# xuyuan/waymo_2d_tracking

Hardware: AMD Instinct MI355X
Metric: end-to-end frames/sec (detect+SORT) on 1920x1280 Waymo frames (higher is better)
Workload: dtype f32; 1 GPU; Cascade R-CNN X152-32x8d-FPN dconv (random-init, fp32, batch 1) on synthetic 1920x1280x3 frames -> top-100 detections/frame -> SORT (max_age 2, min_hits 0, all boxes tracked; trackers resident for the whole segment); 5 cameras x 2 frames per step per GPU; 1x1 and dense 3x3 convolutions: f32 operands as exact 3 x bf16 splits, six cross terms on the bf16 matrix cores, f32 accumulate (csrc/det_gemm_s; stage=e2e, parallelism=sequence-shard x1

## Files before the change

waymo_2d_tracking_amd/csrc/det_deform.hip:

```cpp
#include "common.h"
#include "../../include/waymodet.h"
#include <cstdlib>

namespace {

using f32x4 = __attribute__((ext_vector_type(4))) float;
constexpr int TP = 64;
constexpr int CCH = 128;
constexpr int LDC = CCH + 2;

struct Sample {
    unsigned idx[4];
    float wgt[4];
};

template <int CG, bool DEFORM>
__global__ __launch_bounds__(256, (CG <= 32 ? 3 : 2)) void deform_conv3x3_kernel(
    const float* __restrict__ x, const float* __restrict__ offset, const float* __restrict__ mask,
    const float* __restrict__ wp, const float* __restrict__ scale, const float* __restrict__ bias, int relu,
    int batch, int H, int W, int C, int Cout, int Ho, int Wo, int stride, int pad, float* __restrict__ y) {
    constexpr bool PRIV = CG <= 32;
    constexpr int LDW = PRIV ? 34 : LDC;
    __shared__ Sample tab[TP * 9];
    __shared__ __attribute__((aligned(16))) float col[PRIV ? 4 * TP * 34 : TP * LDC];
    const int tid = threadIdx.x, lane = tid & 63, wave = tid >> 6;
    const int tiles_x = (Wo + 7) >> 3, tiles_y = (Ho + 7) >> 3;
    const int ntiles = batch * tiles_y * tiles_x;
    const int nchunks = C / CCH;
    int tile, chunk;
    {
        const int b = blockIdx.x;
        const int xcd = b & 7, slot = b >> 3;
        if (nchunks >= 8 && (nchunks & 7) == 0) {
            const int cpx = nchunks >> 3;
            chunk = xcd * cpx + slot % cpx;
            tile = slot / cpx;
        } else if (nchunks < 8 && (8 % nchunks) == 0 && (ntiles % (8 / nchunks)) == 0) {
            const int xpc = 8 / nchunks;
            const int tpp = ntiles / xpc;
            chunk = xcd / xpc;
            tile = (xcd % xpc) * tpp + slot;
        } else {
            chunk = b / ntiles;
            tile = b - chunk * ntiles;
        }
    }
    if (tile >= ntiles || chunk >= nchunks) return;
    const int tn = tile / (tiles_y * tiles_x);
    const int trem = tile - tn * tiles_y * tiles_x;
    const int tyy = trem / tiles_x, txx = trem - tyy * tiles_x;
    __shared__ int pix[TP];
    if (tid < TP) {
        const int ho = tyy * 8 + (tid >> 3), wo = txx * 8 + (tid & 7);
        pix[tid] = (ho < Ho && wo < Wo) ? (tn * Ho + ho) * Wo + wo : -1;
    }
    __syncthreads();
    const int c0 = chunk * CCH;
    for (int e = tid; e < TP * 9; e += 256) {
        const int p = e / 9, k = e - 9 * p;
        const long gp = pix[p];
        Sample s;
#pragma unroll
        for (int q = 0; q < 4; ++q) { s.idx[q] = 0u; s.wgt[q] = 0.f; }
        if (gp >= 0) {
            const int n = (int)(gp / ((long)Ho * Wo));
            const int rem = (int)(gp - (long)n * Ho * Wo);
            const int ho = rem / Wo, wo = rem - ho * Wo;
            const int kh = k / 3, kw = k - 3 * kh;
            if (!DEFORM) {
                const int hi = ho * stride - pad + kh, wi = wo * stride - pad + kw;
                if (hi >= 0 && hi < H && wi >= 0 && wi < W) { s.idx[0] = (unsigned)(n * H * W + hi * W + wi) * (unsigned)C * 4u; s.wgt[0] = 1.f; }
                tab[e] = s;
                continue;
            }
            const float* off = offset + (size_t)gp * 18;
            const float h_im = (float)(ho * stride - pad + kh) + off[2 * k];
            const float w_im = (float)(wo * stride - pad + kw) + off[2 * k + 1];
            if (h_im > -1.f && w_im > -1.f && h_im < (float)H && w_im < (float)W) {
                const int hl = (int)floorf(h_im), wl = (int)floorf(w_im);
                const int hh = hl + 1, wh = wl + 1;
                const float lh = h_im - (float)hl, lw = w_im - (float)wl;
                const float uh = 1.f - lh, uw = 1.f - lw;
                const float m = mask ? mask[(size_t)gp * 9 + k] : 1.f;
                const int base = n * H * W;
                if (hl >= 0 && wl >= 0) { s.idx[0] = (unsigned)(base + hl * W + wl) * (unsigned)C * 4u; s.wgt[0] = uh * uw * m; }
                if (hl >= 0 && wh <= W - 1) { s.idx[1] = (unsigned)(base + hl * W + wh) * (unsigned)C * 4u; s.wgt[1] = uh * lw * m; }
                if (hh <= H - 1 && wl >= 0) { s.idx[2] = (unsigned)(base + hh * W + wl) * (unsigned)C * 4u; s.wgt[2] = lh * uw * m; }
                if (hh <= H - 1 && wh <= W - 1) { s.idx[3] = (unsigned)(base + hh * W + wh) * (unsigned)C * 4u; s.wgt[3] = lh * lw * m; }
            }
        }
        tab[e] = s;
    }
    f32x4 acc[4][2];
#pragma unroll
    for (int i = 0; i < 4; ++i)
#pragma unroll
        for (int j = 0; j < 2; ++j) acc[i][j] = (f32x4){0.f, 0.f, 0.f, 0.f};
    __syncthreads();

    const int gq = PRIV ? (lane & 7) : (tid & 31);
    const int gp0 = PRIV ? (lane >> 3) : (tid >> 5);
    const int co_w = wave * 32;
    float* colw = PRIV ? col + wave * (TP * 34) : col;
    auto slab_sync = [&]() {
        if (PRIV) {
            __builtin_amdgcn_fence(__ATOMIC_RELEASE, "wavefront");
            __builtin_amdgcn_wave_barrier();
            __builtin_amdgcn_fence(__ATOMIC_ACQUIRE, "wavefront");
        } else {
            __syncthreads();
        }
    };
    constexpr int NQ = DEFORM ? 4 : 1;
    const char* xb = reinterpret_cast<const char*>(x);
    const unsigned lane_off = (unsigned)(c0 + (PRIV ? co_w : 0) + gq * 4) * 4u;
    float4 tA[4][NQ];
    auto issue = [&](int k, int half, float4 (&t)[4][NQ]) {
#pragma unroll
        for (int i = 0; i < 4; ++i) {
            const int p = gp0 + 8 * (half * 4 + i);
            const Sample& s = tab[p * 9 + k];
#pragma unroll
            for (int q = 0; q < NQ; ++q)
                t[i][q] = *reinterpret_cast<const float4*>(xb + (size_t)(s.idx[q] + lane_off));
        }
    };
    auto blend = [&](int k, int half, const float4 (&t)[4][NQ]) {
#pragma unroll
        for (int i = 0; i < 4; ++i) {
            const int p = gp0 + 8 * (half * 4 + i);
            const Sample& s = tab[p * 9 + k];
            float4 v = make_float4(0.f, 0.f, 0.f, 0.f);
#pragma unroll
            for (int q = 0; q < NQ; ++q) {
                const float wq = s.wgt[q];
                v.x += wq * t[i][q].x; v.y += wq * t[i][q].y;
                v.z += wq * t[i][q].z; v.w += wq * t[i][q].w;
            }
            float2* d = reinterpret_cast<float2*>(&colw[p * LDW + gq * 4]);
            d[0] = make_float2(v.x, v.y);
            d[1] = make_float2(v.z, v.w);
        }
    };
    constexpr int KS = (CG >= 16) ? CG / 4 : 4;
    float bR[2][KS];
    auto load_b = [&](int k) {
#pragma unroll
        for (int nt = 0; nt < 2; ++nt) {
            const int co_l = co_w + 16 * nt;
            if (CG >= 16) {
                const int g = (c0 + co_l) / CG;
                const int co_g = (co_l % CG) + (lane & 15);
                const float* wb = wp + ((size_t)(g * 9 + k) * CG) * CG + co_g;
#pragma unroll
                for (int kk = 0; kk < KS; ++kk) bR[nt][kk] = wb[(size_t)(kk * 4 + (lane >> 4)) * CG];
            } else {
                const int j = lane & 15;
                const int g = (c0 + co_l) / 8 + (j >> 3);
#pragma unroll
                for (int kk = 0; kk < KS; ++kk) {
                    const int ci = kk * 4 + (lane >> 4);
                    const float wv = wp[((size_t)(g * 9 + k) * 8 + (ci & 7)) * 8 + (j & 7)];
                    bR[nt][kk] = ((ci >> 3) == (j >> 3)) ? wv : 0.f;
                }
            }
        }
    };
    issue(0, 0, tA);
    for (int k = 0; k < 9; ++k) {
        blend(k, 0, tA);
        load_b(k);
        {
            float4 tB[4][NQ];
            issue(k, 1, tB);
            __builtin_amdgcn_sched_barrier(0);
            blend(k, 1, tB);
        }
        slab_sync();
        if (k + 1 < 9) issue(k + 1, 0, tA);
        __builtin_amdgcn_sched_barrier(0);
#pragma unroll
        for (int nt = 0; nt < 2; ++nt) {
            const int co_l = co_w + 16 * nt;
            const int cl = PRIV ? 16 * nt : co_l;
            const int a_col = (CG >= 16) ? (cl / CG) * CG : cl;
#pragma unroll
            for (int kk = 0; kk < KS; ++kk) {
                const int ci = kk * 4 + (lane >> 4);
#pragma unroll
                for (int mt = 0; mt < 4; ++mt) {
                    const float a = colw[(mt * 16 + (lane & 15)) * LDW + a_col + ci];
                    acc[mt][nt] = __builtin_amdgcn_mfma_f32_16x16x4f32(a, bR[nt][kk], acc[mt][nt], 0, 0, 0);
                }
            }
        }
        slab_sync();
    }
#pragma unroll
    for (int nt = 0; nt < 2; ++nt) {
        const int co = c0 + co_w + 16 * nt + (lane & 15);
        const float sc = scale ? scale[co] : 1.f;
        const float bi = bias ? bias[co] : 0.f;
#pragma unroll
        for (int mt = 0; mt < 4; ++mt)
#pragma unroll
            for (int r = 0; r < 4; ++r) {
                const long gp = pix[mt * 16 + (lane >> 4) * 4 + r];
                if (gp >= 0) {
                    float v = acc[mt][nt][r] * sc + bi;
                    if (relu) v = fmaxf(v, 0.f);
                    y[(size_t)gp * Cout + co] = v;
                }
            }
    }
}


constexpr int PCH = 64;
constexpr int PR = 2;
constexpr int PS = 10 + 2 * PR;
constexpr int LDP = PCH + 2;

template <int CG>
__global__ __launch_bounds__(256, 2) void deform_conv3x3_patch_kernel(
    const float* __restrict__ x, const float* __restrict__ offset, const float* __restrict__ mask,
    const float* __restrict__ wp, const float* __restrict__ scale, const float* __restrict__ bias, int relu,
    int batch, int H, int W, int C, int Cout, int Ho, int Wo, float* __restrict__ y) {
    __shared__ __attribute__((aligned(16))) float patch[PS * PS * PCH];
    __shared__ __attribute__((aligned(16))) float col[TP * LDP];
    __shared__ float offs[TP * 18];
    __shared__ float msk[TP * 9];
    __shared__ int pix[TP];
    const int tid = threadIdx.x, lane = tid & 63, wave = tid >> 6;
    const int tiles_x = (Wo + 7) >> 3, tiles_y = (Ho + 7) >> 3;
    const int ntiles = batch * tiles_y * tiles_x;
    const int nchunks = C / PCH;
    int tile, chunk;
    {
        const int b = blockIdx.x;
        const int xcd = b & 7, slot = b >> 3;
        if ((nchunks & 7) == 0) {
            const int cpx = nchunks >> 3;
            chunk = xcd * cpx + slot % cpx;
            tile = slot / cpx;
        } else {
            chunk = b / ntiles;
            tile = b - chunk * ntiles;
        }
    }
    if (tile >= ntiles || chunk >= nchunks) return;
    const int tn = tile / (tiles_y * tiles_x);
    const int trem = tile - tn * tiles_y * tiles_x;
    const int tyy = trem / tiles_x, txx = trem - tyy * tiles_x;
    const int c0 = chunk * PCH;
    const int py0 = tyy * 8 - 1 - PR, px0 = txx * 8 - 1 - PR;
    if (tid < TP) {
        const int ho = tyy * 8 + (tid >> 3), wo = txx * 8 + (tid & 7);
        pix[tid] = (ho < Ho && wo < Wo) ? (tn * Ho + ho) * Wo + wo : -1;
    }
    for (int e = tid; e < PS * PS * (PCH / 4); e += 256) {
        const int pp = e >> 4, q = e & 15;
        const int r = pp / PS, cc = pp - r * PS;
        const int iy = py0 + r, ix = px0 + cc;
        float4 v = make_float4(0.f, 0.f, 0.f, 0.f);
        if (iy >= 0 && iy < H && ix >= 0 && ix < W)
            v = *reinterpret_cast<const float4*>(x + ((size_t)(tn * H + iy) * W + ix) * C + c0 + q * 4);
        *reinterpret_cast<float4*>(&patch[pp * PCH + q * 4]) = v;
    }
    __syncthreads();
    for (int e = tid; e < TP * 18; e += 256) {
        const int p = e / 18;
        const int gp = pix[p];
        offs[e] = gp >= 0 ? offset[(size_t)gp * 18 + (e - 18 * p)] : 0.f;
    }
    for (int e = tid; e < TP * 9; e += 256) {
        const int p = e / 9;
        const int gp = pix[p];
        msk[e] = (gp >= 0) ? (mask ? mask[(size_t)gp * 9 + (e - 9 * p)] : 1.f) : 0.f;
    }
    f32x4 acc[4];
#pragma unroll
    for (int i = 0; i < 4; ++i) acc[i] = (f32x4){0.f, 0.f, 0.f, 0.f};
    __syncthreads();

    const int gq = tid & 15;
    const int gp0 = tid >> 4;
    const int co_l = wave * 16;
    const int g_l = co_l / CG;
    const int g = (c0 + co_l) / CG;
    const int co_g = (co_l % CG) + (lane & 15);
    for (int k = 0; k < 9; ++k) {
        const int kh = k / 3, kw = k - 3 * kh;
        float breg[CG / 4];
        {
            const float* wb = wp + ((size_t)(g * 9 + k) * CG) * CG + co_g;
#pragma unroll
            for (int kk = 0; kk < CG / 4; ++kk) breg[kk] = wb[(size_t)(kk * 4 + (lane >> 4)) * CG];
        }
#pragma unroll
        for (int i = 0; i < 4; ++i) {
            const int p = gp0 + 16 * i;
            const float ry = (float)((p >> 3) + kh + PR) + offs[p * 18 + 2 * k];
            const float rx = (float)((p & 7) + kw + PR) + offs[p * 18 + 2 * k + 1];
            const float h_im = ry + (float)py0, w_im = rx + (float)px0;
            const float m = msk[p * 9 + k];
            float4 v = make_float4(0.f, 0.f, 0.f, 0.f);
            if (m != 0.f && h_im > -1.f && w_im > -1.f && h_im < (float)H && w_im < (float)W) {
                const float fy = floorf(ry), fx = floorf(rx);
                const int hl = (int)fy, wl = (int)fx;
                const float lh = ry - fy, lw = rx - fx, uh = 1.f - lh, uw = 1.f - lw;
                if (hl >= 0 && hl < PS - 1 && wl >= 0 && wl < PS - 1) {
                    const float* pb = &patch[(hl * PS + wl) * PCH + gq * 4];
                    const float4 a = *reinterpret_cast<const float4*>(pb);
                    const float4 b = *reinterpret_cast<const float4*>(pb + PCH);
                    const float4 c = *reinterpret_cast<const float4*>(pb + PS * PCH);
                    const float4 d = *reinterpret_cast<const float4*>(pb + PS * PCH + PCH);
                    const float w1 = uh * uw, w2 = uh * lw, w3 = lh * uw, w4 = lh * lw;
                    v.x = w1 * a.x + w2 * b.x + w3 * c.x + w4 * d.x;
                    v.y = w1 * a.y + w2 * b.y + w3 * c.y + w4 * d.y;
                    v.z = w1 * a.z + w2 * b.z + w3 * c.z + w4 * d.z;
                    v.w = w1 * a.w + w2 * b.w + w3 * c.w + w4 * d.w;
                } else {
                    const int ih = hl + py0, iw = wl + px0;
                    const float wq[4] = {uh * uw, uh * lw, lh * uw, lh * lw};
#pragma unroll
                    for (int qd = 0; qd < 4; ++qd) {
                        const int yy = ih + (qd >> 1), xx = iw + (qd & 1);
                        if (yy >= 0 && yy < H && xx >= 0 && xx < W) {
                            const float4 t = *reinterpret_cast<const float4*>(x + ((size_t)(tn * H + yy) * W + xx) * C + c0 + gq * 4);
                            v.x += wq[qd] * t.x; v.y += wq[qd] * t.y; v.z += wq[qd] * t.z; v.w += wq[qd] * t.w;
                        }
                    }
                }
                v.x *= m; v.y *= m; v.z *= m; v.w *= m;
            }
            float2* dd = reinterpret_cast<float2*>(&col[p * LDP + gq * 4]);
            dd[0] = make_float2(v.x, v.y);
            dd[1] = make_float2(v.z, v.w);
        }
        __syncthreads();
#pragma unroll
        for (int kk = 0; kk < CG / 4; ++kk) {
            const int ci = kk * 4 + (lane >> 4);
#pragma unroll
            for (int mt = 0; mt < 4; ++mt) {
                const float a = col[(mt * 16 + (lane & 15)) * LDP + g_l * CG + ci];
                acc[mt] = __builtin_amdgcn_mfma_f32_16x16x4f32(a, breg[kk], acc[mt], 0, 0, 0);
            }
        }
        __syncthreads();
    }
    const int co = c0 + co_l + (lane & 15);
    const float sc = scale ? scale[co] : 1.f;
    const float bi = bias ? bias[co] : 0.f;
#pragma unroll
    for (int mt = 0; mt < 4; ++mt)
#pragma unroll
        for (int r = 0; r < 4; ++r) {
            const long gp = pix[mt * 16 + (lane >> 4) * 4 + r];
            if (gp >= 0) {
                float v = acc[mt][r] * sc + bi;
                if (relu) v = fmaxf(v, 0.f);
                y[(size_t)gp * Cout + co] = v;
            }
        }
}

#define PROW(p) (((p) >> 4) + 4 * (((p) >> 3) & 1))
constexpr int PST = PCH + 4;
template <int CG>
__global__ __launch_bounds__(256, 2) void deform_conv3x3_lds_kernel(
    const float* __restrict__ x, const float* __restrict__ offset, const float* __restrict__ mask,
    const float* __restrict__ wp, const float* __restrict__ scale, const float* __restrict__ bias, int relu,
    int batch, int H, int W, int C, int Cout, int Ho, int Wo, float* __restrict__ y) {
    constexpr int GPW = PCH / CG;
    constexpr int WPG = 4 / GPW;
    constexpr int MT = 4 / WPG;
    constexpr int NT = CG / 16;
    constexpr int KS = CG / 4;
    constexpr int PW = 16 * MT;
    __shared__ __attribute__((aligned(16))) float patch[PS * PS * PST];
    __shared__ __attribute__((aligned(16))) float4 tw[TP * 9];
    __shared__ int toff[TP * 9];
    __shared__ int pix[TP];
    __shared__ int any_fb;
    const int tid = threadIdx.x, lane = tid & 63, wave = tid >> 6;
    const int tiles_x = (Wo + 7) >> 3, tiles_y = (Ho + 7) >> 3;
    const int ntiles = batch * tiles_y * tiles_x;
    const int nchunks = C / PCH;
    int tile, chunk;
    {
        const int b = blockIdx.x;
        const int xcd = b & 7, slot = b >> 3;
        if ((nchunks & 7) == 0) {
            const int cpx = nchunks >> 3;
            chunk = xcd * cpx + slot % cpx;
            tile = slot / cpx;
        } else {
            chunk = b / ntiles;
            tile = b - chunk * ntiles;
        }
    }
    if (tile >= ntiles || chunk >= nchunks) return;
    const int tn = tile / (tiles_y * tiles_x);
    const int trem = tile - tn * tiles_y * tiles_x;
    const int tyy = trem / tiles_x, txx = trem - tyy * tiles_x;
    const int c0 = chunk * PCH;
    const int py0 = tyy * 8 - 1 - PR, px0 = txx * 8 - 1 - PR;
    if (tid == 0) any_fb = 0;
    if (tid < TP) {
        const int ho = tyy * 8 + PROW(tid), wo = txx * 8 + (tid & 7);
        pix[tid] = (ho < Ho && wo < Wo) ? (tn * Ho + ho) * Wo + wo : -1;
    }
    const int g_l = wave / WPG;
    const int p_base = (wave % WPG) * PW;
    const int r16 = lane & 15, kq = lane >> 4;
    const int ch_l = g_l * CG + kq * KS;
    const int g = (c0 + g_l * CG) / CG;
    float bR[2][NT][KS];
    const float* __restrict__ wfrag = wp + (size_t)Cout * CG * 9 + ((size_t)g * 9 * 64 + lane) * (NT * KS);
    auto load_b = [&](int k, float (&b)[NT][KS]) {
        const float4* src = reinterpret_cast<const float4*>(wfrag + (size_t)k * 64 * (NT * KS));
#pragma unroll
        for (int j = 0; j < NT * KS / 4; ++j) {
            const float4 v = src[j];
            b[(4 * j) / KS][(4 * j) % KS + 0] = v.x; b[(4 * j) / KS][(4 * j) % KS + 1] = v.y;
            b[(4 * j) / KS][(4 * j) % KS + 2] = v.z; b[(4 * j) / KS][(4 * j) % KS + 3] = v.w;
        }
    };
    load_b(0, bR[0]);
    constexpr int NE = (TP * 9 + 255) / 256;
    float e_dy[NE], e_dx[NE], e_m[NE];
    int e_gp[NE];
#pragma unroll
    for (int j = 0; j < NE; ++j) {
        const int e = tid + 256 * j;
        const int p = e / 9, k = e - 9 * p;
        int gp = -1;
        if (e < TP * 9) {
            const int ho = tyy * 8 + PROW(p), wo = txx * 8 + (p & 7);
            gp = (ho < Ho && wo < Wo) ? (tn * Ho + ho) * Wo + wo : -1;
        }
        e_gp[j] = gp;
        e_dy[j] = e_dx[j] = 0.f;
        e_m[j] = 1.f;
        if (gp >= 0) {
            e_dy[j] = offset[(size_t)gp * 18 + 2 * k];
            e_dx[j] = offset[(size_t)gp * 18 + 2 * k + 1];
            if (mask) e_m[j] = mask[(size_t)gp * 9 + k];
        }
    }
    {
        constexpr int NL = (PS * PS * (PCH / 4) + 255) / 256;
        float4 v[NL];
#pragma unroll
        for (int j = 0; j < NL; ++j) {
            const int e = tid + 256 * j;
            const int pp = e >> 4, q = e & 15;
            const int r = pp / PS, cc = pp - r * PS;
            const int iy = py0 + r, ix = px0 + cc;
            v[j] = make_float4(0.f, 0.f, 0.f, 0.f);
            if (e < PS * PS * (PCH / 4) && iy >= 0 && iy < H && ix >= 0 && ix < W)
                v[j] = *reinterpret_cast<const float4*>(x + ((size_t)(tn * H + iy) * W + ix) * C + c0 + q * 4);
        }
#pragma unroll
        for (int j = 0; j < NL; ++j) {
            const int e = tid + 256 * j;
            if (e < PS * PS * (PCH / 4)) *reinterpret_cast<float4*>(&patch[(e >> 4) * PST + (e & 15) * 4]) = v[j];
        }
    }
    __syncthreads();
#pragma unroll
    for (int j = 0; j < NE; ++j) {
        const int e = tid + 256 * j;
        if (e >= TP * 9) continue;
        const int p = e / 9, k = e - 9 * p;
        float4 w4 = make_float4(0.f, 0.f, 0.f, 0.f);
        int off = 0;
        if (e_gp[j] >= 0) {
            const int kh = k / 3, kw = k - 3 * kh;
            const float ry = (float)(PROW(p) + kh + PR) + e_dy[j];
            const float rx = (float)((p & 7) + kw + PR) + e_dx[j];
            const float h_im = ry + (float)py0, w_im = rx + (float)px0;
            const float m = e_m[j];
            if (h_im > -1.f && w_im > -1.f && h_im < (float)H && w_im < (float)W) {
                const float fy = floorf(ry), fx = floorf(rx);
                const int hl = (int)fy, wl = (int)fx;
                const float lh = ry - fy, lw = rx - fx, uh = 1.f - lh, uw = 1.f - lw;
                w4 = make_float4(uh * uw * m, uh * lw * m, lh * uw * m, lh * lw * m);
                if (hl >= 0 && hl < PS - 1 && wl >= 0 && wl < PS - 1) {
                    off = (hl * PS + wl) * PST;
                } else {
                    off = -1 - ((hl + py0 + 2) * (W + 4) + (wl + px0 + 2));
                    any_fb = 1;
                }
            }
        }
        tw[e] = w4;
        toff[e] = off;
    }
    f32x4 acc[MT][NT];
#pragma unroll
    for (int i = 0; i < MT; ++i)
#pragma unroll
        for (int j = 0; j < NT; ++j) acc[i][j] = (f32x4){0.f, 0.f, 0.f, 0.f};
    __syncthreads();
    const bool slow = any_fb != 0;

    auto mfma = [&](const float (&a)[MT][KS], const float (&b)[NT][KS]) {
#pragma unroll
        for (int kk = 0; kk < KS; ++kk) {
#pragma unroll
            for (int mt = 0; mt < MT; ++mt)
#pragma unroll
                for (int nt = 0; nt < NT; ++nt)
                    acc[mt][nt] = __builtin_amdgcn_mfma_f32_16x16x4f32(a[mt][kk], b[nt][kk], acc[mt][nt], 0, 0, 0);
        }
    };
    if (!slow) {
        float4 cv[MT][4][KS / 4];
        float4 wv[MT];
        float a[2][MT][KS];
        auto gather_issue = [&](int k) {
#pragma unroll
            for (int mt = 0; mt < MT; ++mt) {
                const int e = (p_base + mt * 16 + r16) * 9 + k;
                const float* pb = &patch[toff[e] + ch_l];
                wv[mt] = tw[e];
#pragma unroll
                for (int h = 0; h < KS / 4; ++h) {
                    cv[mt][0][h] = *reinterpret_cast<const float4*>(pb + 4 * h);
                    cv[mt][1][h] = *reinterpret_cast<const float4*>(pb + PST + 4 * h);
                    cv[mt][2][h] = *reinterpret_cast<const float4*>(pb + PS * PST + 4 * h);
                    cv[mt][3][h] = *reinterpret_cast<const float4*>(pb + PS * PST + PST + 4 * h);
                }
            }
        };
        auto blend = [&](float (&o)[MT][KS]) {
#pragma unroll
            for (int mt = 0; mt < MT; ++mt)
#pragma unroll
                for (int h = 0; h < KS / 4; ++h) {
                    o[mt][4 * h + 0] = wv[mt].x * cv[mt][0][h].x + wv[mt].y * cv[mt][1][h].x + wv[mt].z * cv[mt][2][h].x + wv[mt].w * cv[mt][3][h].x;
                    o[mt][4 * h + 1] = wv[mt].x * cv[mt][0][h].y + wv[mt].y * cv[mt][1][h].y + wv[mt].z * cv[mt][2][h].y + wv[mt].w * cv[mt][3][h].y;
                    o[mt][4 * h + 2] = wv[mt].x * cv[mt][0][h].z + wv[mt].y * cv[mt][1][h].z + wv[mt].z * cv[mt][2][h].z + wv[mt].w * cv[mt][3][h].z;
                    o[mt][4 * h + 3] = wv[mt].x * cv[mt][0][h].w + wv[mt].y * cv[mt][1][h].w + wv[mt].z * cv[mt][2][h].w + wv[mt].w * cv[mt][3][h].w;
                }
        };
        gather_issue(0);
        blend(a[0]);
#pragma unroll
        for (int k = 0; k < 9; ++k) {
            if (k + 1 < 9) load_b(k + 1, bR[(k + 1) & 1]);
            if (k + 1 < 9) gather_issue(k + 1);
            mfma(a[k & 1], bR[k & 1]);
            if (k + 1 < 9) blend(a[(k + 1) & 1]);
            if (k + 1 < 9) {
                constexpr int NM = MT * NT * KS;
                constexpr int NDS = MT * (2 + KS);
                constexpr int H1 = NM / 4;
                __builtin_amdgcn_sched_group_barrier(0x020, NT * KS / 4, 0);
#pragma unroll
                for (int j = 0; j < H1; ++j) {
                    __builtin_amdgcn_sched_group_barrier(0x008, 1, 0);
                    __builtin_amdgcn_sched_group_barrier(0x100, (NDS + H1 - 1) / H1, 0);
                }
#pragma unroll
                for (int j = 0; j < NM / 4; ++j) __builtin_amdgcn_sched_group_barrier(0x008, 1, 0);
#pragma unroll
                for (int j = 0; j < NM - H1 - NM / 4; ++j) {
                    __builtin_amdgcn_sched_group_barrier(0x008, 1, 0);
                    __builtin_amdgcn_sched_group_barrier(0x002, (MT * KS * 4 + (NM - H1 - NM / 4) - 1) / (NM - H1 - NM / 4), 0);
                }
            }
            __builtin_amdgcn_sched_barrier(0);
        }
    } else {
#pragma unroll
        for (int k = 0; k < 9; ++k) {
            if (k + 1 < 9) load_b(k + 1, bR[(k + 1) & 1]);
            float a[MT][KS];
#pragma unroll
            for (int mt = 0; mt < MT; ++mt) {
                const int e = (p_base + mt * 16 + r16) * 9 + k;
                const int off = toff[e];
                const float4 w4 = tw[e];
                const float wq[4] = {w4.x, w4.y, w4.z, w4.w};
#pragma unroll
                for (int kk = 0; kk < KS; ++kk) a[mt][kk] = 0.f;
                if (off >= 0) {
                    const float* pb = &patch[off + ch_l];
#pragma unroll
                    for (int qd = 0; qd < 4; ++qd)
#pragma unroll
                        for (int h = 0; h < KS / 4; ++h) {
                            const float4 t = *reinterpret_cast<const float4*>(pb + (qd >> 1) * PS * PST + (qd & 1) * PST + 4 * h);
                            a[mt][4 * h + 0] += wq[qd] * t.x; a[mt][4 * h + 1] += wq[qd] * t.y;
                            a[mt][4 * h + 2] += wq[qd] * t.z; a[mt][4 * h + 3] += wq[qd] * t.w;
                        }
                } else {
                    const int code = -1 - off;
                    const int ih = code / (W + 4) - 2, iw = code - (ih + 2) * (W + 4) - 2;
#pragma unroll
                    for (int qd = 0; qd < 4; ++qd) {
                        const int yy = ih + (qd >> 1), xx = iw + (qd & 1);
                        if (yy >= 0 && yy < H && xx >= 0 && xx < W) {
                            const float* gb = x + ((size_t)(tn * H + yy) * W + xx) * C + c0 + ch_l;
#pragma unroll
                            for (int h = 0; h < KS / 4; ++h) {
                                const float4 t = *reinterpret_cast<const float4*>(gb + 4 * h);
                                a[mt][4 * h + 0] += wq[qd] * t.x; a[mt][4 * h + 1] += wq[qd] * t.y;
                                a[mt][4 * h + 2] += wq[qd] * t.z; a[mt][4 * h + 3] += wq[qd] * t.w;
                            }
                        }
                    }
                }
            }
            mfma(a, bR[k & 1]);
        }
    }
#pragma unroll
    for (int nt = 0; nt < NT; ++nt) {
        const int co = c0 + g_l * CG + 16 * nt + (lane & 15);
        const float sc = scale ? scale[co] : 1.f;
        const float bi = bias ? bias[co] : 0.f;
#pragma unroll
        for (int mt = 0; mt < MT; ++mt)
#pragma unroll
            for (int r = 0; r < 4; ++r) {
                const long gp = pix[p_base + mt * 16 + (lane >> 4) * 4 + r];
                if (gp >= 0) {
                    float v = acc[mt][nt][r] * sc + bi;
                    if (relu) v = fmaxf(v, 0.f);
                    y[(size_t)gp * Cout + co] = v;
                }
            }
    }
}

__global__ void pack_weight_kernel(const float* __restrict__ w, int cg, int cout, float* __restrict__ packed) {
    const long total = (long)cout * cg * 9;
    for (long e = (long)blockIdx.x * blockDim.x + threadIdx.x; e < total; e += (long)gridDim.x * blockDim.x) {
        const int co = (int)(e % cg);
        const int ci = (int)((e / cg) % cg);
        const int k = (int)((e / ((long)cg * cg)) % 9);
        const int g = (int)(e / ((long)cg * cg * 9));
        const float v = w[(((size_t)(g * cg + co) * cg) + ci) * 9 + k];
        packed[e] = v;
        if (cg == 16 || cg == 32) {
            const int KS = cg / 4, NT = cg / 16;
            const int kq = ci / KS, kk = ci - kq * KS, nt = co >> 4, r16 = co & 15;
            const int lane = kq * 16 + r16;
            packed[total + (((size_t)(g * 9 + k) * 64 + lane) * NT + nt) * KS + kk] = v;
        }
    }
}

}

int wt::victim_regs_deform64() {
    hipFuncAttributes at{};
    if (hipFuncGetAttributes(&at, reinterpret_cast<const void*>(deform_conv3x3_kernel<64, true>)) != hipSuccess) return 0;
    return (at.numRegs + 7) / 8 * 8;
}


int wd_deform_pp_launch(const float* x, const float* offset, const float* packed_weight, const float* scale,
                        const float* bias, int relu, int batch, int h, int w, int c, int cg, int stride, hipStream_t stream, float* y,
                        const void* table);
int wd_grouped_conv3x3_c8_launch(const float* x, const float* packed_weight, const float* scale, const float* bias, int relu,
                                 int batch, int h, int w, int c, hipStream_t stream, float* y);

static int deform_variant(int cg, int stride, int pad, bool has_offset, const char* mode) {
    const bool fits = has_offset && stride == 1 && pad == 1;
    if (mode && strcmp(mode, "none") == 0) return 0;
    if (has_offset && stride == 2 && pad == 1 && (cg == 32 || cg == 16) && !(mode && strcmp(mode, "lds") == 0)) return 3;
    if (mode && strcmp(mode, "all") == 0) return (fits && (cg == 16 || cg == 32 || cg == 64)) ? 1 : 0;
    if (fits && (cg == 32 || cg == 16) && !(mode && strcmp(mode, "lds") == 0)) return 3;
    if (fits && (cg == 16 || cg == 32)) return 2;
    if (fits && cg == 64) return 1;
    return 0;
}

extern "C" {

const char* wd_deform_conv3x3_variant(int c_in, int groups, int stride, int pad, int has_offset) {
    if (groups <= 0 || c_in % groups) return "invalid";
    const int cg = c_in / groups;
    switch (deform_variant(cg, stride, pad, has_offset != 0, getenv("WD_DEFORM_PATCH"))) {
        case 3: return cg == 16 ? "deform_conv3x3_pp_kernel<16>" : "deform_conv3x3_pp_kernel<32>";
        case 2: return cg == 16 ? "deform_conv3x3_lds_kernel<16>" : "deform_conv3x3_lds_kernel<32>";
        case 1: return cg == 16 ? "deform_conv3x3_patch_kernel<16>" : cg == 32 ? "deform_conv3x3_patch_kernel<32>" : "deform_conv3x3_patch_kernel<64>";
        default: break;
    }
    if (!has_offset && cg == 8 && stride == 1 && pad == 1 && (c_in % 128) == 0) return "grouped_conv3x3_c8_kernel";
    if (has_offset) return cg == 8 ? "deform_conv3x3_kernel<8,true>" : cg == 16 ? "deform_conv3x3_kernel<16,true>" : cg == 32 ? "deform_conv3x3_kernel<32,true>" : "deform_conv3x3_kernel<64,true>";
    return cg == 8 ? "deform_conv3x3_kernel<8,false>" : cg == 16 ? "deform_conv3x3_kernel<16,false>" : cg == 32 ? "deform_conv3x3_kernel<32,false>" : "deform_conv3x3_kernel<64,false>";
}

size_t wd_deform_packed_weight_floats(int c_in, int c_out, int groups) {
    if (groups <= 0 || c_in % groups || c_in != c_out) return 0;
    return 2 * (size_t)c_out * (size_t)(c_in / groups) * 9;
}

int wd_deform_pack_weight(const float* weight_oihw, int c_in, int c_out, int groups, float* packed, void* stream) {
    WT_TRY(wt::ensure_device());
    if (!wd_deform_packed_weight_floats(c_in, c_out, groups)) {
        wt::set_error("wd_deform_pack_weight: needs c_in == c_out divisible by groups");
        return WT_ERR_INVALID;
    }
    hipLaunchKernelGGL(pack_weight_kernel, dim3(256), dim3(256), 0, (hipStream_t)stream, weight_oihw, c_in / groups, c_out, packed);
    WT_HIP(hipGetLastError());
    return WT_OK;
}

int wd_deform_conv3x3_f32(const float* x, const float* offset, const float* mask, const float* packed_weight,
                          const float* scale, const float* bias, int relu, int batch, int h, int w, int c_in,
                          int c_out, int groups, int stride, int pad, float* y, void* stream_) {
    return wd_deform_conv3x3_tab_f32(x, offset, mask, packed_weight, scale, bias, relu, batch, h, w, c_in, c_out, groups, stride, pad,
                                     0, nullptr, y, stream_);
}

int wd_deform_conv3x3_hint_f32(const float* x, const float* offset, const float* mask, const float* packed_weight,
                               const float* scale, const float* bias, int relu, int batch, int h, int w, int c_in,
                               int c_out, int groups, int stride, int pad, int far_offsets, float* y, void* stream_) {
    return wd_deform_conv3x3_tab_f32(x, offset, mask, packed_weight, scale, bias, relu, batch, h, w, c_in, c_out, groups, stride, pad,
                                     far_offsets, nullptr, y, stream_);
}

int wd_deform_conv3x3_tab_f32(const float* x, const float* offset, const float* mask, const float* packed_weight,
                              const float* scale, const float* bias, int relu, int batch, int h, int w, int c_in,
                              int c_out, int groups, int stride, int pad, int far_offsets, const void* table, float* y,
                              void* stream_) {
    WT_TRY(wt::ensure_device());
    if (c_in != c_out || groups <= 0 || c_in % groups || c_in % CCH || stride < 1 || batch < 1 || h < 1 || w < 1 ||
        ((uintptr_t)x & 15)) {
        wt::set_error("wd_deform_conv3x3_f32: unsupported shape (c_in=%d c_out=%d groups=%d; need c_in == c_out, c_in %% 128 == 0)",
                      c_in, c_out, groups);
        return WT_ERR_INVALID;
    }
    if ((double)batch * h * w * c_in * 4.0 >= 4294967296.0) {
        wt::set_error("wd_deform_conv3x3_f32: input of %d x %d x %d x %d floats exceeds the kernel's 32-bit byte offsets (4 GiB); "
                      "split the batch", batch, h, w, c_in);
        return WT_ERR_CAPACITY;
    }
    const int cg = c_in / groups;
    const int ho = (h + 2 * pad - 3) / stride + 1, wo = (w + 2 * pad - 3) / stride + 1;
    if (ho < 1 || wo < 1) return WT_OK;
    const long ntiles = (long)batch * ((ho + 7) / 8) * ((wo + 7) / 8);
    const long nwg = ntiles * (c_in / CCH);
    dim3 grid((unsigned)((nwg + 7) / 8 * 8));
    hipStream_t stream = (hipStream_t)stream_;
    const char* mode = getenv("WD_DEFORM_PATCH");
    if (!offset && !mask && cg == 8 && stride == 1 && pad == 1 && (c_in % 128) == 0 && ((uintptr_t)y & 7) == 0)
        return wd_grouped_conv3x3_c8_launch(x, packed_weight, scale, bias, relu, batch, h, w, c_in, stream, y);
    int variant = deform_variant(cg, stride, pad, offset != nullptr, mode);
    if (variant == 3 && stride != 1 && mask) variant = 0;
    if (variant == 3 && stride == 1 && (mask || far_offsets)) variant = 2;
    if (variant == 3)
        return wd_deform_pp_launch(x, offset, packed_weight, scale, bias, relu, batch, h, w, c_in, cg, stride, stream, y, table);
    if (variant == 2) {
        const long nwg_p = ntiles * (c_in / PCH);
        dim3 gridp((unsigned)((nwg_p + 7) / 8 * 8));
        if (cg == 16)
            hipLaunchKernelGGL(deform_conv3x3_lds_kernel<16>, gridp, dim3(256), 0, stream, x, offset, mask, packed_weight, scale,
                               bias, relu, batch, h, w, c_in, c_out, ho, wo, y);
        else
            hipLaunchKernelGGL(deform_conv3x3_lds_kernel<32>, gridp, dim3(256), 0, stream, x, offset, mask, packed_weight, scale,
                               bias, relu, batch, h, w, c_in, c_out, ho, wo, y);
        WT_HIP(hipGetLastError());
        return WT_OK;
    }
    if (variant == 1) {
        const long nwg_p = ntiles * (c_in / PCH);
        dim3 gridp((unsigned)((nwg_p + 7) / 8 * 8));
#define WD_LAUNCH_P(CG)                                                                                              \
    hipLaunchKernelGGL(deform_conv3x3_patch_kernel<CG>, gridp, dim3(256), 0, stream, x, offset, mask, packed_weight, \
                       scale, bias, relu, batch, h, w, c_in, c_out, ho, wo, y)
        if (cg == 16) WD_LAUNCH_P(16);
        else if (cg == 32) WD_LAUNCH_P(32);
        else WD_LAUNCH_P(64);
#undef WD_LAUNCH_P
        WT_HIP(hipGetLastError());
        return WT_OK;
    }
#define WD_LAUNCH(CG)                                                                                                     \
    do {                                                                                                                  \
        if (offset)                                                                                                       \
            hipLaunchKernelGGL((deform_conv3x3_kernel<CG, true>), grid, dim3(256), 0, stream, x, offset, mask,           \
                               packed_weight, scale, bias, relu, batch, h, w, c_in, c_out, ho, wo, stride, pad, y);       \
        else                                                                                                              \
            hipLaunchKernelGGL((deform_conv3x3_kernel<CG, false>), grid, dim3(256), 0, stream, x, offset, mask,          \
                               packed_weight, scale, bias, relu, batch, h, w, c_in, c_out, ho, wo, stride, pad, y);       \
    } while (0)
    if (cg == 16) WD_LAUNCH(16);
    else if (cg == 32) WD_LAUNCH(32);
    else if (cg == 64) WD_LAUNCH(64);
    else if (cg == 8) WD_LAUNCH(8);
    else {
        wt::set_error("wd_deform_conv3x3_f32: channels per group must be 8, 16, 32 or 64 (got %d)", cg);
        return WT_ERR_INVALID;
    }
#undef WD_LAUNCH
    WT_HIP(hipGetLastError());
    return WT_OK;
}

}
```

waymo_2d_tracking_amd/csrc/det_gconv.hip:

```cpp
#include "common.h"
#include <cstdlib>
#include "../../include/waymodet.h"

namespace {

namespace gc {
constexpr int CH = 128;
constexpr int TS = 8;
constexpr int PS = TS + 2;
constexpr int PATCH_F = PS * PS * CH;
}

typedef float float2v __attribute__((ext_vector_type(2)));

__global__ __launch_bounds__(256, 2) void grouped_conv3x3_c8_kernel(const float* __restrict__ x, const float* __restrict__ packed,
                                                                    const float* __restrict__ scale, const float* __restrict__ bias,
                                                                    int relu, int batch, int H, int W, int C, float* __restrict__ y) {
    extern __shared__ __attribute__((aligned(16))) float patch[];
    const int tid = threadIdx.x, lane = tid & 63, wave = __builtin_amdgcn_readfirstlane(tid >> 6);
    const int halves = C / gc::CH;
    const int half = blockIdx.x % halves;
    const int c0 = half * gc::CH;
    const int tiles_x = (W + gc::TS - 1) / gc::TS, tiles_y = (H + gc::TS - 1) / gc::TS;
    const int ntiles = batch * tiles_y * tiles_x;
    const int co = c0 + 2 * lane;
    const int g = co >> 3, col = co & 7;
    float2v wr[9][8];
#pragma unroll
    for (int k = 0; k < 9; ++k)
#pragma unroll
        for (int ci = 0; ci < 8; ++ci) {
            const float2 t = *reinterpret_cast<const float2*>(packed + ((size_t)(g * 9 + k) * 8 + ci) * 8 + col);
            wr[k][ci] = (float2v){t.x, t.y};
        }
    const float2v sc = scale ? (float2v){scale[co], scale[co + 1]} : (float2v){1.f, 1.f};
    const float2v bi = bias ? (float2v){bias[co], bias[co + 1]} : (float2v){0.f, 0.f};
    const int gl = lane >> 2;
    constexpr int NI = gc::PS * gc::PS / 2;
    constexpr int NW = (NI + 3) / 4;
    const int lane_off = ((lane >> 5) * C + (lane & 31) * 4) * 4;
    const char* xb = reinterpret_cast<const char*>(x);
    const int step = gridDim.x / halves;
    for (int t = blockIdx.x / halves; t < ntiles; t += step) {
        const int tn = t / (tiles_y * tiles_x), tr = t - tn * tiles_y * tiles_x;
        const int ty = tr / tiles_x, tx = tr - ty * tiles_x;
        const int y0 = ty * gc::TS - 1, x0 = tx * gc::TS - 1;
        const char* origin = xb + ((((long)tn * H + y0) * W + x0) * C + c0) * 4;
        const bool inner = y0 >= 0 && x0 >= 0 && y0 + gc::PS <= H && x0 + gc::PS <= W;
        __syncthreads();
        {
#pragma unroll
            for (int i = 0; i < NW; ++i) {
                const int j = wave + 4 * i;
                if (j >= NI) continue;
                const int py = (2 * j) / gc::PS, px = 2 * j - py * gc::PS;
                const char* sbase = origin + ((long)py * W + px) * C * 4;
                const unsigned dst = (unsigned)(j * 1024);
                const int iy = y0 + py, ix = x0 + px + (lane >> 5);
                if (inner || (iy >= 0 && iy < H && ix >= 0 && ix < W)) {
                    unsigned keep;
                    asm volatile("s_mov_b32 %0, m0\n\ts_mov_b32 m0, %3\n\ts_nop 0\n\tglobal_load_lds_dwordx4 %1, %2\n\ts_mov_b32 m0, %0"
                                 : "=&s"(keep) : "v"(lane_off), "s"(sbase), "s"(dst) : "memory");
                } else {
                    *reinterpret_cast<float4*>(reinterpret_cast<char*>(patch) + dst + lane * 16) = make_float4(0.f, 0.f, 0.f, 0.f);
                }
            }
        }
        __builtin_amdgcn_s_waitcnt(0x0070);
        __syncthreads();
        constexpr int npix = gc::TS * gc::TS;
        float4 cur[3][2], nxt[3][2];
        auto read_row = [&](int p, int kh, float4 (&dst)[3][2]) {
            const float* src = patch + (((p >> 3) + kh) * gc::PS + (p & 7)) * gc::CH + gl * 8;
#pragma unroll
            for (int kw = 0; kw < 3; ++kw) {
                dst[kw][0] = *reinterpret_cast<const float4*>(src + kw * gc::CH);
                dst[kw][1] = *reinterpret_cast<const float4*>(src + kw * gc::CH + 4);
            }
        };
        read_row(wave, 0, cur);
        for (int p = wave; p < npix; p += 4) {
            float2v acc0 = {0.f, 0.f}, acc1 = {0.f, 0.f}, acc2 = {0.f, 0.f}, acc3 = {0.f, 0.f};
#pragma unroll
            for (int kh = 0; kh < 3; ++kh) {
                if (kh < 2) read_row(p, kh + 1, nxt);
                else read_row((p + 4 < npix) ? p + 4 : p, 0, nxt);
                __builtin_amdgcn_sched_barrier(0);
#pragma unroll
                for (int kw = 0; kw < 3; ++kw) {
                    const int k = kh * 3 + kw;
                    acc0 += wr[k][0] * cur[kw][0].x; acc1 += wr[k][1] * cur[kw][0].y;
                    acc2 += wr[k][2] * cur[kw][0].z; acc3 += wr[k][3] * cur[kw][0].w;
                    acc0 += wr[k][4] * cur[kw][1].x; acc1 += wr[k][5] * cur[kw][1].y;
                    acc2 += wr[k][6] * cur[kw][1].z; acc3 += wr[k][7] * cur[kw][1].w;
                }
                __builtin_amdgcn_sched_barrier(0);
#pragma unroll
                for (int kw = 0; kw < 3; ++kw) { cur[kw][0] = nxt[kw][0]; cur[kw][1] = nxt[kw][1]; }
            }
            const int oy = ty * gc::TS + (p >> 3), ox = tx * gc::TS + (p & 7);
            if (oy < H && ox < W) {
                float2v v = ((acc0 + acc1) + (acc2 + acc3)) * sc + bi;
                if (relu) { v.x = fmaxf(v.x, 0.f); v.y = fmaxf(v.y, 0.f); }
                *reinterpret_cast<float2*>(y + (((size_t)tn * H + oy) * W + ox) * C + co) = make_float2(v.x, v.y);
            }
        }
    }
}

}

int wt::victim_regs_grouped_conv() {
    hipFuncAttributes at{};
    if (hipFuncGetAttributes(&at, reinterpret_cast<const void*>(grouped_conv3x3_c8_kernel)) != hipSuccess) return 0;
    return (at.numRegs + 7) / 8 * 8;
}

int wd_grouped_conv3x3_c8_launch(const float* x, const float* packed_weight, const float* scale, const float* bias, int relu,
                                 int batch, int h, int w, int c, hipStream_t stream, float* y) {
    const int n_cu = wt::device_cus() > 0 ? wt::device_cus() : 256;
    static wt::OncePerDevice attr;
    const int dev = wt::device_index();
    const size_t smem = (size_t)gc::PATCH_F * sizeof(float);
    if (attr.needed(dev)) {
        WT_HIP(hipFuncSetAttribute(reinterpret_cast<const void*>(grouped_conv3x3_c8_kernel), hipFuncAttributeMaxDynamicSharedMemorySize,
                                   (int)smem));
        attr.mark(dev);
    }
    const int halves = c / gc::CH;
    const long ntiles = (long)batch * ((h + gc::TS - 1) / gc::TS) * ((w + gc::TS - 1) / gc::TS);
    long per_half = (2L * n_cu + halves - 1) / halves;
    if (per_half > ntiles) per_half = ntiles;
    if (per_half < 1) per_half = 1;
    hipLaunchKernelGGL(grouped_conv3x3_c8_kernel, dim3((unsigned)(per_half * halves)), dim3(256), smem, stream, x, packed_weight,
                       scale, bias, relu, batch, h, w, c, y);
    WT_HIP(hipGetLastError());
    return WT_OK;
}
```

Baseline: 43.52 frames/s.

## Add MFMA-based grouped 3x3 conv kernel for 8-channel groups with double-buffered patches

Adds a new kernel for the non-deformable grouped 3x3 conv with 8 channels per group. It runs the per-group products on f32 16x16x4 MFMA instructions, using block-diagonal zero-padded weight fragments held in registers. Input patches are double-buffered in LDS with async global-to-LDS loads and XOR swizzling, and the epilogue of the previous tile overlaps the current one. Tiles are split across XCDs with a persistent grid of 512-thread blocks. The cost is wasted MFMA work on the zero blocks, plus a dependence on 16-byte output alignment, which falls back to the old kernel when not met.

```diff
diff --git a/waymo_2d_tracking_amd/csrc/det_deform.hip b/waymo_2d_tracking_amd/csrc/det_deform.hip
--- a/waymo_2d_tracking_amd/csrc/det_deform.hip
+++ b/waymo_2d_tracking_amd/csrc/det_deform.hip
@@ -670,6 +670,8 @@
                         const void* table);
 int wd_grouped_conv3x3_c8_launch(const float* x, const float* packed_weight, const float* scale, const float* bias, int relu,
                                  int batch, int h, int w, int c, hipStream_t stream, float* y);
+int wd_grouped_conv3x3_c8_mfma_launch(const float* x, const float* packed_weight, const float* scale, const float* bias, int relu,
+                                      int batch, int h, int w, int c, hipStream_t stream, float* y);
 
 static int deform_variant(int cg, int stride, int pad, bool has_offset, const char* mode) {
     const bool fits = has_offset && stride == 1 && pad == 1;
@@ -693,7 +695,7 @@
         case 1: return cg == 16 ? "deform_conv3x3_patch_kernel<16>" : cg == 32 ? "deform_conv3x3_patch_kernel<32>" : "deform_conv3x3_patch_kernel<64>";
         default: break;
     }
-    if (!has_offset && cg == 8 && stride == 1 && pad == 1 && (c_in % 128) == 0) return "grouped_conv3x3_c8_kernel";
+    if (!has_offset && cg == 8 && stride == 1 && pad == 1 && (c_in % 128) == 0) return "grouped_conv3x3_c8_mfma_kernel";
     if (has_offset) return cg == 8 ? "deform_conv3x3_kernel<8,true>" : cg == 16 ? "deform_conv3x3_kernel<16,true>" : cg == 32 ? "deform_conv3x3_kernel<32,true>" : "deform_conv3x3_kernel<64,true>";
     return cg == 8 ? "deform_conv3x3_kernel<8,false>" : cg == 16 ? "deform_conv3x3_kernel<16,false>" : cg == 32 ? "deform_conv3x3_kernel<32,false>" : "deform_conv3x3_kernel<64,false>";
 }
@@ -752,6 +754,8 @@
     dim3 grid((unsigned)((nwg + 7) / 8 * 8));
     hipStream_t stream = (hipStream_t)stream_;
     const char* mode = getenv("WD_DEFORM_PATCH");
+    if (!offset && !mask && cg == 8 && stride == 1 && pad == 1 && (c_in % 128) == 0 && ((uintptr_t)y & 15) == 0)
+        return wd_grouped_conv3x3_c8_mfma_launch(x, packed_weight, scale, bias, relu, batch, h, w, c_in, stream, y);
     if (!offset && !mask && cg == 8 && stride == 1 && pad == 1 && (c_in % 128) == 0 && ((uintptr_t)y & 7) == 0)
         return wd_grouped_conv3x3_c8_launch(x, packed_weight, scale, bias, relu, batch, h, w, c_in, stream, y);
     int variant = deform_variant(cg, stride, pad, offset != nullptr, mode);
diff --git a/waymo_2d_tracking_amd/csrc/det_gconv.hip b/waymo_2d_tracking_amd/csrc/det_gconv.hip
--- a/waymo_2d_tracking_amd/csrc/det_gconv.hip
+++ b/waymo_2d_tracking_amd/csrc/det_gconv.hip
@@ -108,6 +108,156 @@
     }
 }
 
+namespace gm {
+constexpr int CH = 128;
+constexpr int TS = 8, PS = TS + 2;
+constexpr int PATCH_B = PS * PS * CH * 4;
+constexpr int NI = PS * PS / 2;
+constexpr int NW = (NI + 7) / 8;
+constexpr int XCDS = 8;
+}
+
+using f32x4 = __attribute__((ext_vector_type(4))) float;
+
+__global__ __launch_bounds__(512) void grouped_conv3x3_c8_mfma_kernel(const float* __restrict__ x, const float* __restrict__ packed,
+                                                                      const float* __restrict__ scale, const float* __restrict__ bias,
+                                                                      int relu, int batch, int H, int W, int C, float* __restrict__ y) {
+    extern __shared__ __attribute__((aligned(16))) char smem_m[];
+    const int tid = threadIdx.x, lane = tid & 63, wave = __builtin_amdgcn_readfirstlane(tid >> 6);
+    const int r16 = lane & 15, kq = lane >> 4;
+    const int halves = C / gm::CH;
+    const int xcd = blockIdx.x % gm::XCDS, rb = blockIdx.x / gm::XCDS;
+    const int half = rb % halves, slot = rb / halves;
+    const int step = gridDim.x / (gm::XCDS * halves);
+    const int tiles_x = (W + gm::TS - 1) / gm::TS, tiles_y = (H + gm::TS - 1) / gm::TS;
+    const int ntiles = batch * tiles_y * tiles_x;
+    const int t_lo = (int)((long)ntiles * xcd / gm::XCDS), t_hi = (int)((long)ntiles * (xcd + 1) / gm::XCDS);
+    int t = t_lo + slot;
+    if (t >= t_hi) return;
+    const int c0 = half * gm::CH, cw = c0 + 16 * wave;
+    float wr[9][4];
+    {
+        const bool nz = (r16 >> 3) == (kq >> 1);
+        const float* wg = packed + (size_t)((cw >> 3) + (r16 >> 3)) * 9 * 64 + (r16 & 7);
+#pragma unroll
+        for (int k = 0; k < 9; ++k)
+#pragma unroll
+            for (int j = 0; j < 4; ++j) {
+                const float v = wg[(k * 8 + ((4 * kq + j) & 7)) * 8];
+                wr[k][j] = nz ? v : 0.f;
+            }
+    }
+    const int co = cw + 4 * kq;
+    float4 sc = make_float4(1.f, 1.f, 1.f, 1.f), bi = make_float4(0.f, 0.f, 0.f, 0.f);
+    if (scale) sc = make_float4(scale[co], scale[co + 1], scale[co + 2], scale[co + 3]);
+    if (bias) bi = make_float4(bias[co], bias[co + 1], bias[co + 2], bias[co + 3]);
+    const int dy = (r16 >= 4 && r16 < 12) ? 1 : 0;
+    const int xx = dy ? r16 - 4 : (r16 < 4 ? r16 : r16 - 8);
+    unsigned roff[3][2];
+#pragma unroll
+    for (int kw = 0; kw < 3; ++kw)
+#pragma unroll
+        for (int par = 0; par < 2; ++par) {
+            const int f = ((xx + kw) & 7) | (((dy + par) & 1) << 3);
+            roff[kw][par] = (unsigned)((dy * gm::PS + xx + kw) * 512 + (((4 * wave + kq) ^ f) << 4));
+        }
+    int loff[gm::NW];
+#pragma unroll
+    for (int i = 0; i < gm::NW; ++i) {
+        const int j = wave + 8 * i;
+        const int py = (2 * j) / gm::PS, px = 2 * j - py * gm::PS + (lane >> 5);
+        const int f = (px & 7) | ((py & 1) << 3);
+        loff[i] = ((lane >> 5) * C + (((lane & 31) ^ f) << 2)) * 4;
+    }
+    const char* xb = reinterpret_cast<const char*>(x);
+    struct TileXY { int tn, ty, tx; };
+    auto tile_of = [&](int tt) {
+        TileXY r;
+        r.tn = tt / (tiles_y * tiles_x);
+        const int tr = tt - r.tn * tiles_y * tiles_x;
+        r.ty = tr / tiles_x;
+        r.tx = tr - r.ty * tiles_x;
+        return r;
+    };
+    auto issue_patch = [&](const TileXY& T, unsigned base) {
+        const int y0 = T.ty * gm::TS - 1, x0 = T.tx * gm::TS - 1;
+        const char* origin = xb + ((((long)T.tn * H + y0) * W + x0) * C + c0) * 4;
+        const bool inner = y0 >= 0 && x0 >= 0 && y0 + gm::PS <= H && x0 + gm::PS <= W;
+#pragma unroll
+        for (int i = 0; i < gm::NW; ++i) {
+            const int j = wave + 8 * i;
+            if (j >= gm::NI) continue;
+            const int py = (2 * j) / gm::PS, px = 2 * j - py * gm::PS;
+            const char* sbase = origin + ((long)py * W + px) * C * 4;
+            const unsigned dst = base + (unsigned)(j * 1024);
+            const int iy = y0 + py, ix = x0 + px + (lane >> 5);
+            if (inner || (iy >= 0 && iy < H && ix >= 0 && ix < W)) {
+                unsigned keep;
+                asm volatile("s_mov_b32 %0, m0\n\ts_mov_b32 m0, %3\n\ts_nop 0\n\tglobal_load_lds_dwordx4 %1, %2\n\ts_mov_b32 m0, %0"
+                             : "=&s"(keep) : "v"(loff[i]), "s"(sbase), "s"(dst) : "memory");
+            } else {
+                *reinterpret_cast<float4*>(smem_m + dst + lane * 16) = make_float4(0.f, 0.f, 0.f, 0.f);
+            }
+        }
+    };
+    using lds4 = const __attribute__((address_space(3))) f32x4*;
+    f32x4 acc[4], done[4];
+    TileXY cur = tile_of(t), prev = cur;
+    bool have_prev = false;
+    unsigned base_cur = 0u, base_nxt = (unsigned)gm::PATCH_B;
+    auto epilogue = [&]() {
+#pragma unroll
+        for (int pb = 0; pb < 4; ++pb) {
+            const int oy = prev.ty * gm::TS + 2 * pb + dy, ox = prev.tx * gm::TS + xx;
+            if (oy < H && ox < W) {
+                float4 v;
+                v.x = done[pb][0] * sc.x + bi.x; v.y = done[pb][1] * sc.y + bi.y;
+                v.z = done[pb][2] * sc.z + bi.z; v.w = done[pb][3] * sc.w + bi.w;
+                if (relu) { v.x = fmaxf(v.x, 0.f); v.y = fmaxf(v.y, 0.f); v.z = fmaxf(v.z, 0.f); v.w = fmaxf(v.w, 0.f); }
+                *reinterpret_cast<float4*>(y + (((size_t)prev.tn * H + oy) * W + ox) * C + co) = v;
+            }
+        }
+    };
+    issue_patch(cur, base_cur);
+    for (;;) {
+        __builtin_amdgcn_s_waitcnt(0x0070);
+        __syncthreads();
+        const int t_nxt = t + step;
+        const bool have_next = t_nxt < t_hi;
+        TileXY nxt = cur;
+        if (have_next) { nxt = tile_of(t_nxt); issue_patch(nxt, base_nxt); }
+        if (have_prev) epilogue();
+        f32x4 rd[2][4];
+        auto read_tap = [&](int k, f32x4 (&dst)[4]) {
+            const int kh = k / 3, kw = k - 3 * kh;
+            const unsigned a = base_cur + roff[kw][kh & 1] + (unsigned)(kh * gm::PS * 512);
+#pragma unroll
+            for (int pb = 0; pb < 4; ++pb) dst[pb] = *(lds4)(uintptr_t)(a + (unsigned)(2 * pb * gm::PS * 512));
+        };
+#pragma unroll
+        for (int pb = 0; pb < 4; ++pb) acc[pb] = (f32x4){0.f, 0.f, 0.f, 0.f};
+        read_tap(0, rd[0]);
+#pragma unroll
+        for (int k = 0; k < 9; ++k) {
+            if (k < 8) read_tap(k + 1, rd[(k + 1) & 1]);
+            __builtin_amdgcn_sched_barrier(0);
+#pragma unroll
+            for (int j = 0; j < 4; ++j)
+#pragma unroll
+                for (int pb = 0; pb < 4; ++pb)
+                    acc[pb] = __builtin_amdgcn_mfma_f32_16x16x4f32(wr[k][j], rd[k & 1][pb][j], acc[pb], 0, 0, 0);
+            __builtin_amdgcn_sched_barrier(0);
+        }
+#pragma unroll
+        for (int pb = 0; pb < 4; ++pb) done[pb] = acc[pb];
+        prev = cur; have_prev = true;
+        if (!have_next) break;
+        cur = nxt; t = t_nxt;
+        const unsigned tb = base_cur; base_cur = base_nxt; base_nxt = tb;
+    }
+    epilogue();
+}
+
 }
 
 int wt::victim_regs_grouped_conv() {
@@ -137,3 +287,23 @@
     WT_HIP(hipGetLastError());
     return WT_OK;
 }
+
+int wd_grouped_conv3x3_c8_mfma_launch(const float* x, const float* packed_weight, const float* scale, const float* bias, int relu,
+                                      int batch, int h, int w, int c, hipStream_t stream, float* y) {
+    const int n_cu = wt::device_cus() > 0 ? wt::device_cus() : 256;
+    static wt::OncePerDevice attr;
+    const int dev = wt::device_index();
+    const size_t smem = 2 * (size_t)gm::PATCH_B;
+    if (attr.needed(dev)) {
+        WT_HIP(hipFuncSetAttribute(reinterpret_cast<const void*>(grouped_conv3x3_c8_mfma_kernel), hipFuncAttributeMaxDynamicSharedMemorySize,
+                                   (int)smem));
+        attr.mark(dev);
+    }
+    const int unit = gm::XCDS * (c / gm::CH);
+    int grid = n_cu / unit * unit;
+    if (grid < unit) grid = unit;
+    hipLaunchKernelGGL(grouped_conv3x3_c8_mfma_kernel, dim3((unsigned)grid), dim3(512), smem, stream, x, packed_weight, scale, bias, relu,
+                       batch, h, w, c, y);
+    WT_HIP(hipGetLastError());
+    return WT_OK;
+}
```

Result: no change. 43.59 frames/s (median of 5 runs) (+0.2%).
